# nebula-beta/MonocularSfM

Hardware: AMD Instinct MI355X
Metric: descriptor-pairs/sec (and image-pairs/sec); match-index bit-parity vs CPU (higher is better)
Workload: dtype f32

## Files before the change

monocularsfm_amd/csrc/msfm_job.hip.h:

```cpp
#pragma once

static int call_prologue(msfm_ctx* ctx) {
    HIPCHK(ctx, hipSetDevice(ctx->device));
    ctx->cur = &ctx->sc[0];
    for (Scratch& s : ctx->sc) forget_sweeps(ctx, s);
    if (!ctx->deferred.empty()) {
        HIPCHK(ctx, hipDeviceSynchronize());
        ctx->deferred.flush();
    }
    return settle_store(ctx);
}

template <class Attempt>
static int rerun_alone(msfm_ctx* ctx, Attempt attempt) {
    for (int k = 1;; ++k) {
        bool retry = false;
        const int rc = attempt(&retry);
        if (rc != MSFM_OK || !retry) return rc;
        if (k >= 6) return fail(ctx, MSFM_E_DEVICE, "batch kept overflowing its queues");
    }
}

struct MatchJob {
    msfm_ctx* ctx = nullptr;
    std::vector<int32_t> pairs_own;
    const int32_t* pairs = nullptr;
    int n_pairs = 0;
    msfm_match_params prm = {0.8f, 1, 0.7};
    PruneParams prune = {1, 0.8f, 0.7f};
    msfm_verify_params verify_store = {};
    const msfm_verify_params* verify = nullptr;
    bool streaming = false;
    bool select = false;
    bool pose = false;
    bool refine = false;
    hipEvent_t ev_begin = nullptr, ev_end = nullptr;
    int kSets = kInFlight;
    long long kScratchBytes = 1;
    MsfmRouteKnobs knobs = {};
    int kMaxPairsPerBatch = kDefaultMaxPairsPerBatch;
    std::vector<long long> marks;
    long long cost_done = 0;
    bool need_fix = false;
    SubBatch sb[kInFlight];
    int next_begin = 0;
    long long issued = 0, completed = 0;
    bool memory_wait = false;
    int memory_shrinks = 0;

    int start(msfm_ctx* c, const int32_t* pairs_in, int n, const msfm_match_params* params, const msfm_verify_params* vp, bool stream_mode) {
        ctx = c;
        pairs = pairs_in;
        n_pairs = n;
        streaming = stream_mode;
        verify = nullptr;
        c->have_results = c->sel_valid = c->tv_valid = false;
        select = vp && c->model_select && c->verify_model != MSFM_VERIFY_HOMOGRAPHY;
        c->sel_records.assign(select && !stream_mode ? 3 * (size_t)n : 0, 0);
        pose = vp && c->two_view && c->verify_model == MSFM_VERIFY_ESSENTIAL;
        c->tv_records.assign(pose && !stream_mode ? (size_t)n : 0, msfm_two_view_record{});
        c->tvr_valid = false;
        refine = pose && c->tv_refine;
        c->tvr_records.assign(refine && !stream_mode ? (size_t)n : 0, msfm_two_view_refinement{});
        if (vp) {
            verify_store = *vp;
            verify = &verify_store;
            c->staged_solved = 0;
            c->staged_rounds = 0;
        }
        for (SubBatch& w : sb) w = SubBatch{};
        next_begin = 0;
        issued = completed = 0;
        memory_wait = false;
        memory_shrinks = 0;
        ctx->last_hip_error = 0;
        prm = msfm_match_params{0.8f, 1, 0.7};
        if (params) prm = *params;
        prune = PruneParams{1, prm.ratio, (float)prm.max_distance};
        if ((double)prune.max_distance < prm.max_distance) prune.max_distance = nextafterf(prune.max_distance, __builtin_huge_valf());
        if (!(prm.ratio > 0.f) || !(prm.ratio <= 1.f)) prune.ratio = 0.f;
        if (!(prm.max_distance >= 0.0)) prune.max_distance = __builtin_huge_valf();
        int rc = call_prologue(ctx);
        if (rc != MSFM_OK) return rc;
        rc = rebuild_stale_twins(ctx, pairs, 2 * n_pairs);
        if (rc != MSFM_OK) return rc;
        ctx->res_offsets.assign((size_t)n_pairs + 1, 0);
        ctx->res_sens.assign((size_t)n_pairs, 0);
        ctx->res_count = 0;
        ctx->prof = msfm_profile{};
        ctx->out_used = 0;
        for (OutSeg& s : ctx->out_segs) s.count = 0;
        if (!streaming) {
            long long bound = 1;
            for (int k = 0; k < n_pairs; ++k) {
                const int i = pairs[2 * k], j = pairs[2 * k + 1];
                if (i < 0 || i >= kSlots || j < 0 || j >= kSlots) return fail(ctx, MSFM_E_INVALID, "image id out of range");
                const long long n1 = ctx->images[(size_t)i].n, n2 = ctx->images[(size_t)j].n;
                if (n1 > 0 && n2 > 0) bound += prm.cross_check ? std::min(n1, n2) : n1;
            }
            if (ctx->res_qt.reserve((size_t)bound * 8) != hipSuccess || ctx->res_dist.reserve((size_t)bound * 4) != hipSuccess)
                return fail(ctx, MSFM_E_DEVICE, "cannot reserve address space for the result lists");
        }

        ev_begin = get_event(ctx, 0), ev_end = get_event(ctx, 1);
        if (!ev_begin || !ev_end) return fail(ctx, MSFM_E_DEVICE, "hipEventCreate failed");
        HIPCHK(ctx, hipEventRecord(ev_begin, ctx->sc[0].stream));

        kSets = ctx->in_flight;
        long long budget = ctx->scratch_bytes > 0 ? ctx->scratch_bytes : kDefaultScratchBytes;
        if (ctx->budget_cached > 0 && ctx->budget_for_store == ctx->store.bytes() && ctx->budget_for_limit == ctx->scratch_bytes) {
            budget = ctx->budget_cached;
        } else {
            size_t free_b = 0, total_b = 0;
            if (hipMemGetInfo(&free_b, &total_b) == hipSuccess) {
                long long held = 0;
                for (Scratch& sc : ctx->sc) held += sc.device_bytes();
                const long long avail = (long long)free_b + held;
                budget = std::min(budget, ctx->scratch_bytes > 0 ? avail / 2 : avail / 4);
            }
            ctx->budget_cached = budget;
            ctx->budget_for_store = ctx->store.bytes();
            ctx->budget_for_limit = ctx->scratch_bytes;
        }
        kScratchBytes = std::max<long long>(1, budget / kSets);
        knobs = ctx->route_knobs();
        kMaxPairsPerBatch = ctx->max_pairs_per_batch;
        marks.clear();
        if (ctx->pipeline > 1 && n_pairs > 1) {
            long long total = 0;
            for (int k = 0; k < n_pairs; ++k) {
                const int i = pairs[2 * k], j = pairs[2 * k + 1];
                if (i < 0 || i >= kSlots || j < 0 || j >= kSlots) return fail(ctx, MSFM_E_INVALID, "image id out of range");
                const long long n1 = ctx->images[i].n, n2 = ctx->images[j].n;
                if (n1 > 0 && n2 > 0) total += n1 * n2;
            }
            marks = msfm_pipeline_marks(total, std::min<long long>(ctx->pipeline, total / kMinPipelineCost), ctx->pipeline_taper);
        }
        cost_done = 0;
        need_fix = !(prm.ratio <= 1.f);
        if (streaming) ctx->series_open = true;
        return MSFM_OK;
    }

    int build(SubBatch& w, int begin, const std::vector<char>& force_exact) {
        w.b = Batch{};
        w.begin = begin;
        if (begin == 0) cost_done = 0;
        const long long cost_begin = (begin == w.begin_of_cost) ? w.cost_begin : cost_done;
        w.begin_of_cost = begin;
        w.cost_begin = cost_begin;
        long long mark = 0;
        if (!marks.empty()) {
            size_t i = 0;
            while (i + 2 < marks.size() && cost_begin >= (marks[i] + marks[i + 1]) / 2) ++i;
            mark = marks[i + 1];
        }
        long long est = 0, cost = 0;
        int end = begin;
        while (end < n_pairs && (end - begin) < kMaxPairsPerBatch) {
            PairDesc pd;
            PfPair pp;
            int rc = fill_pair(ctx, pairs[2 * end], pairs[2 * end + 1], pd, pp);
            if (rc != MSFM_OK) return rc;
            const Image &ia = ctx->images[pairs[2 * end]], &ib = ctx->images[pairs[2 * end + 1]];
            if (verify && (ia.nk < ia.n || ib.nk < ib.n))
                return fail(ctx, MSFM_E_STATE, "geometric verification needs msfm_upload_keypoints for image " +
                                                   std::to_string(ia.nk < ia.n ? pairs[2 * end] : pairs[2 * end + 1]));
            const int route = msfm_scratch_route(knobs, prune.prune, prune.ratio, pp.use != 0, ia.is_u8, ib.is_u8);
            const long long need = pd.valid ? msfm_pair_scratch_bytes(pd.n1, pd.n2, pd.n1pad, pd.n2pad, pd.a_blocks, pd.a_blocks256, route, pose, refine) : 0;
            const long long c = pd.valid ? (long long)pd.n1 * pd.n2 : 0;
            if (end > begin && est + need > kScratchBytes) break;
            if (end > begin && !marks.empty() && cost_begin + cost + c / 2 > mark) break;
            est += need;
            cost += c;
            const size_t k = w.b.pairs.size();
            if (k < force_exact.size() && force_exact[k]) {
                pp.use = 0;
                pd.path = 0;
            }
            w.b.pairs.push_back(pd);
            w.b.pf.push_back(pp);
            w.b.id1.push_back(pairs[2 * end]);
            w.b.id2.push_back(pairs[2 * end + 1]);
            ++end;
        }
        w.end = end;
        cost_done = cost_begin + cost;
        return prepare_batch_images(ctx, w.b, prune);
    }

    int issue(SubBatch& w, size_t ev_base) {
        Batch& b = w.b;
        const size_t P = b.pairs.size();
        const int begin = w.begin;
        w.ev_base = ev_base;
        w.exact_launched = false;
        SC.prof = msfm_profile{};
        SC.seq = ctx->issue_seq++;
        SC.sweep2_recorded = false;
        int rc = run_knn(ctx, b, ev_base, &w.exact_launched, prune, need_fix, true);
        if (rc != MSFM_OK) return rc;
        const long long oe = std::max<long long>(1, b.out_elems);
        HIPCHK(ctx, SC.d_st_qt.ensure(oe * sizeof(int2)));
        HIPCHK(ctx, SC.d_st_d.ensure(oe * 4));
        HIPCHK(ctx, SC.d_sub_qt.ensure(oe * sizeof(int2)));
        HIPCHK(ctx, SC.d_sub_d.ensure(oe * 4));
        HIPCHK(ctx, SC.d_counts.ensure(P * 4));
        HIPCHK(ctx, SC.d_sens.ensure(P * 4));
        HIPCHK(ctx, SC.d_offsets.ensure((P + 1) * 8));
        EpiParams ep = {prm.ratio, prm.cross_check, prm.max_distance};
        if (SC.keys_epilogue)
            hipLaunchKernelGGL(epilogue_kernel<KnnFromKeys>, dim3((unsigned)P), dim3(256), 0, SC.stream, SC.d_pairs.as<PairDesc>(), ep,
                               KnnFromKeys{SC.d_tu.as<float>(), SC.d_best.as<unsigned long long>(), SC.d_second.as<unsigned long long>(),
                                           msfm_ratio_cap_on(prune.prune, prune.ratio) ? 1 : 0},
                               SC.d_st_qt.as<int2>(), SC.d_st_d.as<float>(), SC.d_counts.as<int>(), SC.d_sens.as<int>());
        else
            hipLaunchKernelGGL(epilogue_kernel<KnnFromArrays>, dim3((unsigned)P), dim3(256), 0, SC.stream, SC.d_pairs.as<PairDesc>(), ep,
                               KnnFromArrays{SC.d_k_i0.as<int>(), SC.d_k_d0.as<float>(), SC.d_k_d1.as<float>()},
                               SC.d_st_qt.as<int2>(), SC.d_st_d.as<float>(), SC.d_counts.as<int>(), SC.d_sens.as<int>());
        HIPCHK(ctx, hipGetLastError());
        const int* d_counts = SC.d_counts.as<int>();
        const int2* d_st_qt = SC.d_st_qt.as<int2>();
        const float* d_st_d = SC.d_st_d.as<float>();
        if (verify) {
            rc = issue_verify(b, begin, oe, ev_base);
            if (rc != MSFM_OK) return rc;
            d_counts = SC.d_counts2.as<int>();
            d_st_qt = SC.d_st2_qt.as<int2>();
            d_st_d = SC.d_st2_d.as<float>();
        }
        hipLaunchKernelGGL(scan_counts_kernel, dim3(1), dim3(256), 0, SC.stream, d_counts,
                           SC.d_offsets.as<long long>(), (int)P);
        HIPCHK(ctx, hipGetLastError());
        hipLaunchKernelGGL(gather_kernel, dim3((unsigned)P), dim3(256), 0, SC.stream, SC.d_pairs.as<PairDesc>(),
                           d_counts, SC.d_offsets.as<long long>(), d_st_qt,
                           d_st_d, SC.d_sub_qt.as<int2>(), SC.d_sub_d.as<float>());
        HIPCHK(ctx, hipGetLastError());
        rc = queue_tail_copies(ctx, P, select ? &SC.d_vs_records : nullptr);
        if (rc != MSFM_OK) return rc;
        if (pose) {
            const size_t rec_bytes = P * sizeof(msfm_two_view_record);
            HIPCHK(ctx, SC.h_tv.ensure(rec_bytes + (refine ? P * sizeof(msfm_two_view_refinement) : 0) + 64, 0));
            char* h = nullptr;
            HIPCHK(ctx, hipHostGetDevicePointer((void**)&h, SC.h_tv.p, 0));
            ExportSegs segs = {};
            segs.s[0] = ExportSeg{SC.d_tv_records.as<char>(), h, (unsigned)rec_bytes};
            if (refine)
                segs.s[1] = ExportSeg{SC.d_tvr_records.as<char>(), h + rec_bytes, (unsigned)(P * sizeof(msfm_two_view_refinement))};
            hipLaunchKernelGGL(export_tail_kernel, dim3(32), dim3(256), 0, SC.stream, segs);
            HIPCHK(ctx, hipGetLastError());
        }
        return MSFM_OK;
    }

    bool staged() const { return ctx->verify_model == MSFM_VERIFY_ESSENTIAL || ctx->verify_model == MSFM_VERIFY_HOMOGRAPHY; }

    int issue_verify(Batch& b, int begin, long long oe, size_t ev_base) {
        const size_t P = b.pairs.size();
        const int model = ctx->verify_model;
        std::vector<VerifyPair>& vpairs = b.verify_pairs;
        vpairs.resize(P);
        for (size_t p = 0; p < P; ++p)
            vpairs[p] = VerifyPair{ctx->images[pairs[2 * (begin + (int)p)]].kxy, ctx->images[pairs[2 * (begin + (int)p) + 1]].kxy};
        HIPCHK(ctx, SC.d_vf_pairs.ensure(P * sizeof(VerifyPair)));
        const bool e = model == MSFM_VERIFY_ESSENTIAL;
        for (DevBuf* xy : {e ? &SC.d_ve_x1 : &SC.d_vf_x1, e ? &SC.d_ve_y1 : &SC.d_vf_y1, e ? &SC.d_ve_x2 : &SC.d_vf_x2, e ? &SC.d_ve_y2 : &SC.d_vf_y2})
            HIPCHK(ctx, xy->ensure(oe * (e ? 8 : 4)));
        if (select && e)
            for (DevBuf* xy : {&SC.d_vf_x1, &SC.d_vf_y1, &SC.d_vf_x2, &SC.d_vf_y2}) HIPCHK(ctx, xy->ensure(oe * 4));
        if (!staged()) HIPCHK(ctx, SC.d_vf_flags.ensure(oe));
        HIPCHK(ctx, SC.d_vf_hyp.ensure(P * (size_t)verify->max_iters * 4));
        HIPCHK(ctx, SC.d_vf_best_it.ensure(P * 4));
        HIPCHK(ctx, SC.d_vf_best_count.ensure(P * 4));
        if (staged() || select) {
            HIPCHK(ctx, SC.d_staged_state.ensure((3 * P + 2) * 4));
            HIPCHK(ctx, SC.d_staged_stats.ensure(sizeof(StagedStats)));
        }
        if (select) HIPCHK(ctx, SC.d_vs_records.ensure(P * sizeof(SelectRecord)));
        HIPCHK(ctx, SC.d_st2_qt.ensure(oe * sizeof(int2)));
        HIPCHK(ctx, SC.d_st2_d.ensure(oe * 4));
        HIPCHK(ctx, SC.d_counts2.ensure(P * 4));
        HIPCHK(ctx, hipMemcpyAsync(SC.d_vf_pairs.p, vpairs.data(), P * sizeof(VerifyPair), hipMemcpyHostToDevice, SC.stream));
        if (staged() || select) {
            HIPCHK(ctx, hipMemsetAsync(SC.d_staged_state.p, 0, (3 * P + 2) * 4, SC.stream));
            HIPCHK(ctx, hipMemsetAsync(SC.d_staged_stats.p, 0, sizeof(StagedStats), SC.stream));
        }
        hipEvent_t v0 = get_event(ctx, ev_base + 6), v1 = get_event(ctx, ev_base + 7);
        if (!v0 || !v1) return fail(ctx, MSFM_E_DEVICE, "hipEventCreate failed");
        HIPCHK(ctx, hipEventRecord(v0, SC.stream));
        const PairDesc* dp = SC.d_pairs.as<PairDesc>();
        const VerifyPair* vp = SC.d_vf_pairs.as<VerifyPair>();
        const int* d_counts = SC.d_counts.as<int>();
        const int2* d_st_qt = SC.d_st_qt.as<int2>();
        const float* d_st_d = SC.d_st_d.as<float>();
        int* hyp = SC.d_vf_hyp.as<int>();
        const int* best_it = SC.d_vf_best_it.as<int>();
        if (model == MSFM_VERIFY_FUNDAMENTAL) {
            VerifyParams vprm = {verify->threshold * verify->threshold, verify->confidence, verify->max_iters, 0, verify->seed};
            float *x1 = SC.d_vf_x1.as<float>(), *y1 = SC.d_vf_y1.as<float>(), *x2 = SC.d_vf_x2.as<float>(), *y2 = SC.d_vf_y2.as<float>();
            hipLaunchKernelGGL(vf_points_kernel, dim3((unsigned)P), dim3(256), 0, SC.stream, dp, vp, d_counts, d_st_qt, x1, y1, x2, y2);
            HIPCHK(ctx, hipGetLastError());
            hipLaunchKernelGGL(vf_hypotheses_kernel, dim3((unsigned)((vprm.max_iters + 255) / 256), (unsigned)P), dim3(256), 0, SC.stream,
                               dp, d_counts, (const float*)x1, (const float*)y1, (const float*)x2, (const float*)y2, hyp, vprm);
            HIPCHK(ctx, hipGetLastError());
            hipLaunchKernelGGL(vf_select_kernel, dim3((unsigned)((P + 63) / 64)), dim3(64), 0, SC.stream, d_counts, (const int*)hyp, (int)P,
                               vprm, SC.d_vf_best_it.as<int>(), SC.d_vf_best_count.as<int>());
            HIPCHK(ctx, hipGetLastError());
            hipLaunchKernelGGL(vf_mask_compact_kernel, dim3((unsigned)P), dim3(256), 0, SC.stream, dp, d_counts, d_st_qt, d_st_d,
                               (const float*)x1, (const float*)y1, (const float*)x2, (const float*)y2, best_it,
                               (const int*)SC.d_vf_best_count.as<int>(), SC.d_vf_flags.as<unsigned char>(), vprm, SC.d_st2_qt.as<int2>(),
                               SC.d_st2_d.as<float>(), SC.d_counts2.as<int>());
        } else if (model == MSFM_VERIFY_ESSENTIAL) {
            const double f = (ctx->camera.fx + ctx->camera.fy) * 0.5, tn = verify->threshold / f;
            StagedParams prm = {tn * tn, verify->confidence, verify->max_iters, 0, verify->seed};
            double *x1 = SC.d_ve_x1.as<double>(), *y1 = SC.d_ve_y1.as<double>(), *x2 = SC.d_ve_x2.as<double>(), *y2 = SC.d_ve_y2.as<double>();
            hipLaunchKernelGGL(ve_points_kernel, dim3((unsigned)P), dim3(256), 0, SC.stream, dp, vp, d_counts, d_st_qt, ctx->camera, x1, y1, x2, y2);
            HIPCHK(ctx, hipGetLastError());
            int rc = issue_rounds<5, kVeRound>(P, kVeGroupsPerCU, prm, [&](unsigned grid, int* list, StagedStats* stats) {
                hipLaunchKernelGGL(ve_round_kernel, dim3(grid), dim3(kVeRound), 0, SC.stream, dp, d_counts, (const double*)x1, (const double*)y1,
                                   (const double*)x2, (const double*)y2, list, (int)P, hyp, prm, stats);
            });
            if (rc != MSFM_OK) return rc;
            hipLaunchKernelGGL(ve_mask_compact_kernel, dim3((unsigned)P), dim3(64), 0, SC.stream, dp, d_counts, d_st_qt, d_st_d, (const double*)x1,
                               (const double*)y1, (const double*)x2, (const double*)y2, best_it, prm, SC.d_st2_qt.as<int2>(),
                               SC.d_st2_d.as<float>(), SC.d_counts2.as<int>());
        } else {
            StagedParams prm = {verify->threshold * verify->threshold, verify->confidence, verify->max_iters, 0, verify->seed};
            float *x1 = SC.d_vf_x1.as<float>(), *y1 = SC.d_vf_y1.as<float>(), *x2 = SC.d_vf_x2.as<float>(), *y2 = SC.d_vf_y2.as<float>();
            hipLaunchKernelGGL(vf_points_kernel, dim3((unsigned)P), dim3(256), 0, SC.stream, dp, vp, d_counts, d_st_qt, x1, y1, x2, y2);
            HIPCHK(ctx, hipGetLastError());
            int rc = issue_rounds<4, kVhRound>(P, kVhGroupsPerCU, prm, [&](unsigned grid, int* list, StagedStats* stats) {
                hipLaunchKernelGGL(vh_round_kernel, dim3(grid), dim3(kVhRound), 0, SC.stream, dp, d_counts, (const float*)x1, (const float*)y1,
                                   (const float*)x2, (const float*)y2, list, (int)P, hyp, prm, stats);
            });
            if (rc != MSFM_OK) return rc;
            hipLaunchKernelGGL(vh_mask_compact_kernel, dim3((unsigned)P), dim3(64), 0, SC.stream, dp, d_counts, d_st_qt, d_st_d, (const float*)x1,
                               (const float*)y1, (const float*)x2, (const float*)y2, best_it, prm, SC.d_st2_qt.as<int2>(),
                               SC.d_st2_d.as<float>(), SC.d_counts2.as<int>());
        }
        HIPCHK(ctx, hipGetLastError());
        if (pose) {
            HIPCHK(ctx, SC.d_tv_records.ensure(P * sizeof(msfm_two_view_record)));
            HIPCHK(ctx, SC.d_tv_idx.ensure(oe * 4));
            HIPCHK(ctx, SC.d_tv_angles.ensure(oe * 8));
            if (select) {
                HIPCHK(ctx, SC.d_tv_best_it.ensure(P * 4));
                ExportSegs segs = {};
                segs.s[0] = ExportSeg{SC.d_vf_best_it.as<char>(), SC.d_tv_best_it.as<char>(), (unsigned)(P * 4)};
                hipLaunchKernelGGL(export_tail_kernel, dim3(32), dim3(256), 0, SC.stream, segs);
                HIPCHK(ctx, hipGetLastError());
            }
        }
        if (select) {
            const int rc = issue_select(P, dp, vp);
            if (rc != MSFM_OK) return rc;
        }
        if (pose) {
            const double f = (ctx->camera.fx + ctx->camera.fy) * 0.5, tn = verify->threshold / f;
            const StagedParams prm = {tn * tn, verify->confidence, verify->max_iters, 0, verify->seed};
            const unsigned grid = (unsigned)std::min<size_t>(P, (size_t)kTvGroupsPerCU * (size_t)std::max(1, ctx->cu_count));
            hipLaunchKernelGGL(tv_pose_kernel, dim3(grid), dim3(kTvThreads), 0, SC.stream, dp, d_counts, (const double*)SC.d_ve_x1.as<double>(),
                               (const double*)SC.d_ve_y1.as<double>(), (const double*)SC.d_ve_x2.as<double>(),
                               (const double*)SC.d_ve_y2.as<double>(), (const int*)(select ? SC.d_tv_best_it.as<int>() : SC.d_vf_best_it.as<int>()),
                               (const SelectRecord*)(select ? SC.d_vs_records.as<SelectRecord>() : nullptr), prm, f, ctx->tv_params, (int)P,
                               SC.d_tv_idx.as<int>(), SC.d_tv_angles.as<double>(), SC.d_tv_records.as<msfm_two_view_record>());
            HIPCHK(ctx, hipGetLastError());
            if (refine) {
                HIPCHK(ctx, SC.d_tvr_records.ensure(P * sizeof(msfm_two_view_refinement)));
                const unsigned rgrid = (unsigned)std::min<size_t>(P, (size_t)kTvrGroupsPerCU * (size_t)std::max(1, ctx->cu_count));
                hipLaunchKernelGGL(tv_refine_kernel, dim3(rgrid), dim3(kTvrThreads), 0, SC.stream, dp, (const double*)SC.d_ve_x1.as<double>(),
                                   (const double*)SC.d_ve_y1.as<double>(), (const double*)SC.d_ve_x2.as<double>(),
                                   (const double*)SC.d_ve_y2.as<double>(), (const int*)SC.d_tv_idx.as<int>(), f, ctx->tv_params,
                                   ctx->tvr_params, (int)P, SC.d_tv_angles.as<double>(), SC.d_tv_records.as<msfm_two_view_record>(),
                                   SC.d_tvr_records.as<msfm_two_view_refinement>());
                HIPCHK(ctx, hipGetLastError());
            }
        }
        HIPCHK(ctx, hipEventRecord(v1, SC.stream));
        return MSFM_OK;
    }

    int issue_select(size_t P, const PairDesc* dp, const VerifyPair* vp) {
        StagedParams prm = {verify->threshold * verify->threshold, verify->confidence, verify->max_iters, 0, verify->seed};
        const int* d_counts = SC.d_counts.as<int>();
        const int2* d_st_qt = SC.d_st_qt.as<int2>();
        const float* d_st_d = SC.d_st_d.as<float>();
        int* hyp = SC.d_vf_hyp.as<int>();
        float *x1 = SC.d_vf_x1.as<float>(), *y1 = SC.d_vf_y1.as<float>(), *x2 = SC.d_vf_x2.as<float>(), *y2 = SC.d_vf_y2.as<float>();
        if (ctx->verify_model == MSFM_VERIFY_ESSENTIAL) {
            hipLaunchKernelGGL(vf_points_kernel, dim3((unsigned)P), dim3(256), 0, SC.stream, dp, vp, d_counts, d_st_qt, x1, y1, x2, y2);
            HIPCHK(ctx, hipGetLastError());
        }
        HIPCHK(ctx, hipMemsetAsync(SC.d_staged_state.p, 0, (3 * P + 2) * 4, SC.stream));
        int rc = issue_rounds<4, kVhRound>(P, kVhGroupsPerCU, prm, [&](unsigned grid, int* list, StagedStats* stats) {
            hipLaunchKernelGGL(vh_round_kernel, dim3(grid), dim3(kVhRound), 0, SC.stream, dp, d_counts, (const float*)x1, (const float*)y1,
                               (const float*)x2, (const float*)y2, list, (int)P, hyp, prm, stats);
        });
        if (rc != MSFM_OK) return rc;
        hipLaunchKernelGGL(two_view_select_kernel, dim3((unsigned)P), dim3(64), 0, SC.stream, dp, d_counts, d_st_qt, d_st_d, (const float*)x1,
                           (const float*)y1, (const float*)x2, (const float*)y2, (const int*)SC.d_vf_best_it.as<int>(), prm, ctx->verify_model,
                           ctx->h_ratio, SC.d_st2_qt.as<int2>(), SC.d_st2_d.as<float>(), SC.d_counts2.as<int>(),
                           SC.d_vs_records.as<SelectRecord>());
        HIPCHK(ctx, hipGetLastError());
        return MSFM_OK;
    }

    template <int kSample, int kRound, class LaunchRound>
    int issue_rounds(size_t P, int groups_per_cu, StagedParams& prm, LaunchRound launch_round) {
        StagedStats* stats = SC.d_staged_stats.as<StagedStats>();
        int* state = SC.d_staged_state.as<int>();
        int* list = state + P;
        const int rounds = (prm.max_iters + kRound - 1) / kRound;
        const unsigned grid = (unsigned)std::min<size_t>(P, (size_t)groups_per_cu * (size_t)std::max(1, ctx->cu_count));
        for (int r = -1; r < rounds; ++r) {
            prm.round = r;
            if (r >= 0) {
                launch_round(grid, list, stats);
                HIPCHK(ctx, hipGetLastError());
            }
            hipLaunchKernelGGL((staged_decide_kernel<kSample, kRound>), dim3((unsigned)((P + 63) / 64)), dim3(64), 0, SC.stream,
                               (const int*)SC.d_counts.as<int>(), (const int*)SC.d_vf_hyp.as<int>(), (int)P, prm, state, list,
                               SC.d_vf_best_it.as<int>(), SC.d_vf_best_count.as<int>(), stats);
            HIPCHK(ctx, hipGetLastError());
        }
        return MSFM_OK;
    }

    int complete(SubBatch& w, std::vector<char>& force_exact, bool* retry_out) {
        Batch& b = w.b;
        const size_t P = b.pairs.size();
        *retry_out = false;
        HIPCHK(ctx, hipStreamSynchronize(SC.stream));
        bool retry = false, retry_pf = false;
        force_exact.resize(P, 0);
        int rc = check_fix_overflow(ctx, &retry);
        if (rc != MSFM_OK) return rc;
        rc = finish_prefilter(ctx, b, force_exact, &retry_pf);
        if (rc != MSFM_OK) return rc;
        if (retry || retry_pf) {
            ctx->prof.tie_queue_regrows += SC.prof.tie_queue_regrows;
            ctx->prof.plan_regrows += SC.prof.plan_regrows;
            ctx->prof.fallback_pairs += SC.prof.fallback_pairs;
            *retry_out = true;
            return MSFM_OK;
        }
        SC.prof.fallback_pairs = 0;
        const char* h = SC.h_tail.as<char>();
        const long long* offs = reinterpret_cast<const long long*>(h + 8);
        const int32_t* sens = reinterpret_cast<const int32_t*>(h + 8 + (P + 1) * 8);
        const long long total = offs[P];
        const size_t base = streaming ? 0 : ctx->res_count;
        if (ctx->tracks.open && !ctx->tracks.closed && !ctx->tracks.suppress && !ctx->tracks.add_only) {
            rc = tk_fold_sub_batch(ctx, SC, b.id1.data(), b.id2.data(), P, offs);
            if (rc != MSFM_OK) return rc;
        }
        if (streaming) {
            HIPCHK(ctx, SC.h_sub_qt.ensure(((size_t)total + 1) * 8, 0));
            HIPCHK(ctx, SC.h_sub_d.ensure(((size_t)total + 1) * 4, 0));
            if (total > 0) {
                HIPCHK(ctx, hipMemcpyAsync(SC.h_sub_qt.p, SC.d_sub_qt.p, (size_t)total * 8, hipMemcpyDeviceToHost, SC.stream));
                HIPCHK(ctx, hipMemcpyAsync(SC.h_sub_d.p, SC.d_sub_d.p, (size_t)total * 4, hipMemcpyDeviceToHost, SC.stream));
                HIPCHK(ctx, hipStreamSynchronize(SC.stream));
            }
            w.offsets.assign(offs, offs + P + 1);
            w.sens.assign(sens, sens + P);
            if (select) w.sel.assign(sens + P, sens + 4 * P);
            else w.sel.clear();
            if (pose) w.tv.assign(SC.h_tv.as<msfm_two_view_record>(), SC.h_tv.as<msfm_two_view_record>() + P);
            else w.tv.clear();
            w.tvr.clear();
            if (refine) {
                const msfm_two_view_refinement* h_tvr = reinterpret_cast<const msfm_two_view_refinement*>(SC.h_tv.as<msfm_two_view_record>() + P);
                w.tvr.assign(h_tvr, h_tvr + P);
            }
            for (size_t p = 0; p < P; ++p) SC.prof.order_sensitive_rows += sens[p];
            ctx->res_count += (size_t)total;
        } else {
            const size_t need = base + (size_t)total + 1;
            if (ctx->res_qt.ensure_pinned(need * 8) != hipSuccess || ctx->res_dist.ensure_pinned(need * 4) != hipSuccess)
                return fail(ctx, MSFM_E_DEVICE, "cannot page-lock the result lists (beyond the reserved range or the host's memory): use msfm_match_pairs_begin / _next");
            if (total > 0) {
                OutSeg* seg = ctx->out_used ? &ctx->out_segs[ctx->out_used - 1] : nullptr;
                if (!seg || seg->cap - seg->count < (size_t)total) {
                    while (true) {
                        if (ctx->out_used == ctx->out_segs.size()) {
                            ctx->out_segs.push_back(OutSeg{});
                            OutSeg& s = ctx->out_segs.back();
                            const size_t cap = std::max<size_t>((size_t)total * 8, (size_t)4 << 20);
                            HIPCHK(ctx, s.qt.ensure(cap * 8));
                            HIPCHK(ctx, s.d.ensure(cap * 4));
                            s.cap = cap;
                        }
                        seg = &ctx->out_segs[ctx->out_used++];
                        seg->first = base;
                        seg->count = 0;
                        if (seg->cap >= (size_t)total) break;
                    }
                }
                HIPCHK(ctx, ctx->res_qt.copy_in(base * 8, SC.d_sub_qt.p, (size_t)total * 8, SC.stream));
                HIPCHK(ctx, ctx->res_dist.copy_in(base * 4, SC.d_sub_d.p, (size_t)total * 4, SC.stream));
                HIPCHK(ctx, hipMemcpyAsync(seg->qt.as<int2>() + seg->count, SC.d_sub_qt.p, (size_t)total * 8, hipMemcpyDeviceToDevice, SC.stream));
                HIPCHK(ctx, hipMemcpyAsync(seg->d.as<float>() + seg->count, SC.d_sub_d.p, (size_t)total * 4, hipMemcpyDeviceToDevice, SC.stream));
                seg->count += (size_t)total;
            }
            ctx->res_count = base + (size_t)total;
            for (size_t p = 0; p < P; ++p) {
                ctx->res_offsets[(size_t)w.begin + p + 1] = (int64_t)base + offs[p + 1];
                ctx->res_sens[(size_t)w.begin + p] = sens[p];
                SC.prof.order_sensitive_rows += sens[p];
            }
            if (select) std::memcpy(ctx->sel_records.data() + 3 * (size_t)w.begin, sens + P, P * 12);
            if (pose) std::memcpy(ctx->tv_records.data() + (size_t)w.begin, SC.h_tv.p, P * sizeof(msfm_two_view_record));
            if (refine)
                std::memcpy(ctx->tvr_records.data() + (size_t)w.begin, SC.h_tv.as<msfm_two_view_record>() + P, P * sizeof(msfm_two_view_refinement));
        }
        SC.prof.descriptor_pairs += b.desc_pairs;
        SC.prof.dist_algo_bytes += b.algo_bytes;
        rc = accumulate_kernel_time(ctx, w.ev_base, w.exact_launched);
        if (rc != MSFM_OK) return rc;
        if (verify) {
            float vms = 0.f;
            HIPCHK(ctx, hipEventElapsedTime(&vms, ctx->ev_pool[w.ev_base + 6], ctx->ev_pool[w.ev_base + 7]));
            SC.prof.verify_ms += vms;
            if (staged() || select) {
                StagedStats st = {};
                HIPCHK(ctx, hipMemcpyAsync(&st, SC.d_staged_stats.p, sizeof(st), hipMemcpyDeviceToHost, SC.stream));
                HIPCHK(ctx, hipStreamSynchronize(SC.stream));
                ctx->staged_solved += (long long)st.solved;
                ctx->staged_rounds = std::max(ctx->staged_rounds, st.rounds);
            }
        }
        SC.prof.sub_batches += 1;
        add_profile(ctx->prof, SC.prof);
        return MSFM_OK;
    }

// ... 103 lines not shown
```

monocularsfm_amd/csrc/msfm_kernels.hip.h:

```cpp
#pragma once
#include <hip/hip_runtime.h>
#include <stdint.h>
#include "msfm_hostutil.h"

#pragma clang fp contract(off)

namespace msfm {

constexpr int kDim = 128;
constexpr int kBM = 128;
constexpr int kBN = 128;
constexpr int kTM = 8;
constexpr int kTN = 4;
constexpr int kThreads = 512;
constexpr int kChunkPos = 32;
constexpr int kChunks = kDim / kChunkPos;
constexpr int kPanelFloats = kBM * kDim;
constexpr int kSlotFloats = kChunkPos * kBN;
constexpr int kWaveCols = kBN / 8;
constexpr int kWaveSlotFloats = kChunkPos * kWaveCols;
constexpr int kLdsA = 0;
constexpr int kLdsB = kPanelFloats;
constexpr int kLdsFloats = kLdsB + 8 * 2 * kWaveSlotFloats;
constexpr int kLdsBytes = kLdsFloats * 4;
// ... 170 lines not shown
template <int ORDER>
__global__ __launch_bounds__(kThreads) void dist_top2_kernel(
    const PairDesc* __restrict__ pairs, const WorkItem* __restrict__ items,
    float* __restrict__ rp_s0, int* __restrict__ rp_i0, float* __restrict__ rp_s1,
    float* __restrict__ cp_s0, int* __restrict__ cp_i0, float* __restrict__ cp_s1) {
    using OT = OrderTraits<ORDER>;
    extern __shared__ __attribute__((aligned(16))) float smem[];
    float* sA = smem + kLdsA;

    const WorkItem item = items[blockIdx.x];
    if (item.pair < 0) return;
    const PairDesc pd = pairs[item.pair];

    const int tid = threadIdx.x;
    const int lane = tid & 63;
    const int wave = __builtin_amdgcn_readfirstlane(tid >> 6);
    const int ty = lane & 15;
    const int tx = lane >> 4;
    float* sBw = smem + kLdsB + wave * (2 * kWaveSlotFloats);

    const int n_steps = (item.bt_end - item.bt_begin) * kChunks;
    const float* gB = pd.b_panel + (size_t)item.bt_begin * kPanelFloats + wave * kWaveCols + (lane >> 2) * kBN + (lane & 3) * 4;
    auto dma_chunk = [&](int st) {
        const float* g = gB + (size_t)st * kSlotFloats;
        float* l = sBw + (st & 1) * kWaveSlotFloats;
        __builtin_amdgcn_global_load_lds((const __attribute__((address_space(1))) void*)g,
                                         (__attribute__((address_space(3))) void*)l, 16, 0, 0);
        __builtin_amdgcn_global_load_lds((const __attribute__((address_space(1))) void*)(g + 16 * kBN),
                                         (__attribute__((address_space(3))) void*)(l + 256), 16, 0, 0);
    };

    glds_copy(pd.a_panel + (size_t)item.a_blk * kPanelFloats, sA, kPanelFloats, tid);
    dma_chunk(0);
    __syncthreads();

    const int arow0 = item.a_blk * kBM + 4 * ty;
    float r_s0[kTM], r_s1[kTM];
    int r_i0[kTM];
#pragma unroll
    for (int i = 0; i < kTM; ++i) { r_s0[i] = f_inf(); r_s1[i] = f_inf(); r_i0[i] = -1; }
    constexpr bool kStashIdx = OT::kGroups == 16;
    int* sIdx = reinterpret_cast<int*>(smem + kLdsFloats);
    if (kStashIdx) {
#pragma unroll
        for (int i = 0; i < kTM; ++i) sIdx[i * kThreads + tid] = -1;
    }

    v2f lvl0[4][kTN], lvl1[4][kTN], lvl2[4][kTN];
    (void)lvl2;

    int step = 0;
    auto begin_chunk = [&](int c, const float*& sa, const float*& sb) {
        asm volatile("s_waitcnt vmcnt(0)" ::: "memory");
        if (step + 1 < n_steps) dma_chunk(step + 1);
        sa = sA + c * kChunkPos * kBM + 4 * ty;
        sb = sBw + (step & 1) * kWaveSlotFloats + 4 * tx;
        ++step;
    };
#define MSFM_FOREACH(expr)                       \
    _Pragma("unroll") for (int i = 0; i < 4; ++i) \
        _Pragma("unroll") for (int j = 0; j < kTN; ++j) { expr; }

#pragma unroll 1
    for (int bt = item.bt_begin; bt < item.bt_end; ++bt) {
        const float *sa, *sb;
        if (OT::kGroups == 4) {
#pragma unroll 1
            for (int c = 0; c < kChunks; ++c) {
                begin_chunk(c, sa, sb);
                v2f s[4][kTN];
                group_chains<ORDER>(sa, sb, s);
                if ((c & 1) == 0) { MSFM_FOREACH(lvl0[i][j] = s[i][j]) }
                else if (c == 1) { MSFM_FOREACH(lvl1[i][j] = lvl0[i][j] + s[i][j]) }
                else { MSFM_FOREACH(lvl1[i][j] = lvl1[i][j] + (lvl0[i][j] + s[i][j])) }
            }
        } else if (OT::kGroups == 16) {
#pragma unroll 1
            for (int c = 0; c < kChunks; ++c) {
                begin_chunk(c, sa, sb);
                v2f s[4][kTN], q[4][kTN];
                group_chains<ORDER>(sa, sb, lvl0);
                group_chains<ORDER>(sa + OT::kGroupPos * kBM, sb + OT::kGroupPos * kWaveCols, s);
                MSFM_FOREACH(q[i][j] = lvl0[i][j] + s[i][j])
                group_chains<ORDER>(sa + 2 * OT::kGroupPos * kBM, sb + 2 * OT::kGroupPos * kWaveCols, lvl0);
                group_chains<ORDER>(sa + 3 * OT::kGroupPos * kBM, sb + 3 * OT::kGroupPos * kWaveCols, s);
                MSFM_FOREACH(q[i][j] = q[i][j] + (lvl0[i][j] + s[i][j]))
                if (c == 0 || c == 2) { MSFM_FOREACH(lvl1[i][j] = q[i][j]) }
                else if (c == 1) { MSFM_FOREACH(lvl2[i][j] = lvl1[i][j] + q[i][j]) }
                else { MSFM_FOREACH(lvl2[i][j] = lvl2[i][j] + (lvl1[i][j] + q[i][j])) }
            }
        } else {
#pragma unroll 1
            for (int c = 0; c < kChunks; ++c) {
                begin_chunk(c, sa, sb);
                group_chains<ORDER>(sa, sb, lvl0);
                v2f s[4][kTN];
                group_chains<ORDER>(sa + OT::kGroupPos * kBM, sb + OT::kGroupPos * kWaveCols, s);
                if (c == 0 || c == 2) { MSFM_FOREACH(lvl1[i][j] = lvl0[i][j] + s[i][j]) }
                else if (c == 1) { MSFM_FOREACH(lvl2[i][j] = lvl1[i][j] + (lvl0[i][j] + s[i][j])) }
                else { MSFM_FOREACH(lvl2[i][j] = lvl2[i][j] + (lvl1[i][j] + (lvl0[i][j] + s[i][j]))) }
            }
        }
        float fin[kTM][kTN];
#pragma unroll
        for (int i = 0; i < kTM; ++i)
#pragma unroll
            for (int j = 0; j < kTN; ++j)
                fin[i][j] = fminf((OT::kGroups == 4) ? lvl1[i >> 1][j][i & 1] : lvl2[i >> 1][j][i & 1], f_inf());

        const int col0 = bt * kBN + wave * kWaveCols + tx * kTN;
        if ((bt + 1) * kBN > pd.n2 || (item.a_blk + 1) * kBM > pd.n1) {
#pragma unroll
            for (int i = 0; i < kTM; ++i)
#pragma unroll
                for (int j = 0; j < kTN; ++j)
                    if (arow0 + (i & 3) + (i >> 2) * 64 >= pd.n1 || col0 + j >= pd.n2) fin[i][j] = f_inf();
        }
        if (kStashIdx) {
#pragma unroll
            for (int i = 0; i < kTM; ++i) r_i0[i] = sIdx[i * kThreads + tid];
        }
#pragma unroll
        for (int i = 0; i < kTM; ++i)
#pragma unroll
            for (int j = 0; j < kTN; ++j) top2_push(r_s0[i], r_i0[i], r_s1[i], fin[i][j], col0 + j);
        if (kStashIdx) {
#pragma unroll
            for (int i = 0; i < kTM; ++i) sIdx[i * kThreads + tid] = r_i0[i];
        }
#pragma unroll
        for (int j = 0; j < kTN; ++j) {
            float c_s0 = f_inf(), c_s1 = f_inf();
            int c_i0 = -1;
#pragma unroll
            for (int i = 0; i < kTM; ++i)
                top2_push(c_s0, c_i0, c_s1, fin[i][j], arow0 + (i & 3) + (i >> 2) * 64);
#pragma unroll
            for (int m = 1; m < 16; m <<= 1) {
                const float o_s0 = __shfl_xor(c_s0, m);
                const int o_i0 = __shfl_xor(c_i0, m);
                const float o_s1 = __shfl_xor(c_s1, m);
                top2_merge(c_s0, c_i0, c_s1, o_s0, o_i0, o_s1);
            }
            if (ty == 0) {
                const long long o = pd.cp_off + (long long)item.a_blk * pd.n2pad + col0 + j;
                cp_s0[o] = c_s0;
                cp_i0[o] = c_i0;
                cp_s1[o] = c_s1;
            }
        }
    }

    if (kStashIdx) {
#pragma unroll
        for (int i = 0; i < kTM; ++i) r_i0[i] = sIdx[i * kThreads + tid];
    }
#pragma unroll
    for (int i = 0; i < kTM; ++i) {
#pragma unroll
        for (int m = 16; m < 64; m <<= 1) {
            const float o_s0 = __shfl_xor(r_s0[i], m);
            const int o_i0 = __shfl_xor(r_i0[i], m);
            const float o_s1 = __shfl_xor(r_s1[i], m);
            top2_merge(r_s0[i], r_i0[i], r_s1[i], o_s0, o_i0, o_s1);
        }
    }
    __syncthreads();
    float* sR = smem + kLdsB;
    if (tx == 0) {
#pragma unroll
        for (int i = 0; i < kTM; ++i) {
            const int r = 4 * ty + (i & 3) + (i >> 2) * 64;
            sR[(wave * 3 + 0) * kBM + r] = r_s0[i];
            sR[(wave * 3 + 1) * kBM + r] = __int_as_float(r_i0[i]);
            sR[(wave * 3 + 2) * kBM + r] = r_s1[i];
        }
    }
    __syncthreads();
    if (tid < kBM) {
        float s0 = sR[0 * kBM + tid];
        int i0 = __float_as_int(sR[1 * kBM + tid]);
        float s1 = sR[2 * kBM + tid];
#pragma unroll
        for (int w = 1; w < 8; ++w)
            top2_merge(s0, i0, s1, sR[(w * 3 + 0) * kBM + tid], __float_as_int(sR[(w * 3 + 1) * kBM + tid]),
                       sR[(w * 3 + 2) * kBM + tid]);
        const long long o = pd.rp_off + (long long)item.range * pd.n1pad + item.a_blk * kBM + tid;
        rp_s0[o] = s0;
        rp_i0[o] = i0;
        rp_s1[o] = s1;
    }
#undef MSFM_FOREACH
}

__global__ void merge_knn_kernel(const PairDesc* __restrict__ pairs,
                                 const float* __restrict__ rp_s0, const int* __restrict__ rp_i0,
                                 const float* __restrict__ rp_s1, const float* __restrict__ cp_s0,
                                 const int* __restrict__ cp_i0, const float* __restrict__ cp_s1,
                                 int* __restrict__ k_i0, float* __restrict__ k_d0, float* __restrict__ k_d1,
                                 int* __restrict__ fix_count, int4* __restrict__ fix_list, int fix_cap) {
    MSFM_TAIL_PRIO();
    const PairDesc pd = pairs[blockIdx.y];
    if (!pd.valid || pd.path != 0) return;
    const int e = blockIdx.x * blockDim.x + threadIdx.x;
    for (int dir = 0; dir < 2; ++dir) {
        const int n = dir == 0 ? pd.n1 : pd.n2;
        if (e >= n) continue;
        const int npad = dir == 0 ? pd.n1pad : pd.n2pad;
        const int parts = dir == 0 ? pd.ranges : pd.a_blocks;
        const long long base = (dir == 0 ? pd.rp_off : pd.cp_off) + e;
        const float* ps0 = dir == 0 ? rp_s0 : cp_s0;
        const int* pi0 = dir == 0 ? rp_i0 : cp_i0;
        const float* ps1 = dir == 0 ? rp_s1 : cp_s1;
        float s0 = ps0[base], s1 = ps1[base];
        int i0 = pi0[base];
        for (int p = 1; p < parts; ++p) {
            const long long o = base + (long long)p * npad;
            top2_merge(s0, i0, s1, ps0[o], pi0[o], ps1[o]);
        }
        const float d0 = (s0 < f_inf()) ? sqrtf(s0) : 3.402823466e+38f;
        const float d1 = (s1 < f_inf()) ? sqrtf(s1) : 3.402823466e+38f;
        if (!(s0 < f_inf())) i0 = -1;
        const long long ko = (dir == 0 ? pd.kf_off : pd.kr_off) + e;
        k_i0[ko] = i0;
        k_d0[ko] = d0;
        k_d1[ko] = d1;
        if (i0 >= 0 && d0 == d1) {
            const int slot = atomicAdd(fix_count, 1);
            if (slot < fix_cap) fix_list[slot] = make_int4((int)blockIdx.y, dir, e, 0);
        }
    }
}

__device__ __forceinline__ int tie_rawp_pos(int k) { return 64 * (k >> 6) + 4 * (k & 15) + ((k >> 4) & 3); }

template <int ORDER>
__device__ float l2sqr_rowmajor(const float* __restrict__ a, const float* __restrict__ b) {
    using OT = OrderTraits<ORDER>;
    float lvl[5] = {0.f, 0.f, 0.f, 0.f, 0.f};
    for (int g = 0; g < OT::kGroups; ++g) {
        float s = 0.f;
        for (int v = 0; v < 4; ++v) {
            float p = 0.f;
            for (int it = 0; it < OT::kIters; ++it) {
                const int k = tie_rawp_pos(OT::pos_to_k(g * OT::kGroupPos + v * OT::kIters + it));
                const float t = a[k] - b[k];
                if (it == 0) p = t * t;
                else if (OT::kFused) p = __builtin_fmaf(t, t, p);
                else p = p + t * t;
            }
            s = (v == 0) ? p : s + p;
        }
        int j = 0;
        for (int gg = g; gg & 1; gg >>= 1, ++j) s = lvl[j] + s;
        lvl[j] = s;
    }
    return lvl[OT::kGroups == 4 ? 2 : (OT::kGroups == 8 ? 3 : 4)];
}

template <int ORDER>
__global__ void tie_fixup_kernel(const PairDesc* __restrict__ pairs, const int* __restrict__ fix_count,
                                 const int4* __restrict__ fix_list, int fix_cap,
                                 int* __restrict__ k_i0, const float* __restrict__ k_d0) {
    MSFM_TAIL_PRIO();
    const int nfix = min(*fix_count, fix_cap);
    for (int f = blockIdx.x; f < nfix; f += gridDim.x) {
        const int4 w = fix_list[f];
        const PairDesc pd = pairs[w.x];
        const bool fwd = (w.y == 0);
        const float* me = (fwd ? pd.a_rawp : pd.b_rawp) + (size_t)w.z * kDim;
        const float* other = fwd ? pd.b_rawp : pd.a_rawp;
        const int n_other = fwd ? pd.n2 : pd.n1;
        const long long ko = (fwd ? pd.kf_off : pd.kr_off) + w.z;
        const float d0 = k_d0[ko];
        int best = 0x7fffffff;
        for (int t = threadIdx.x; t < n_other; t += 64) {
            const float s = fwd ? l2sqr_rowmajor<ORDER>(me, other + (size_t)t * kDim)
                                : l2sqr_rowmajor<ORDER>(other + (size_t)t * kDim, me);
            if (sqrtf(s) == d0) { best = t; break; }
        }
#pragma unroll
        for (int m = 32; m >= 1; m >>= 1) best = min(best, __shfl_xor(best, m));
        if (threadIdx.x == 0 && best != 0x7fffffff) k_i0[ko] = best;
    }
}

struct EpiParams {
    float ratio;
    int cross_check;
    double max_distance;
};

__device__ __forceinline__ bool order_sensitive(int i0, float d0, float d1, float ratio, double max_distance, bool forward) {
    return msfm_order_sensitive(i0, d0, d1, ratio, max_distance, forward);
}
__device__ __forceinline__ bool lowe_keep(int i0, float d0, float d1, float ratio) {
    return (i0 >= 0) && (d1 < kNoNeighbour || d1 == f_inf()) && (d0 < ratio * d1);
}

struct KnnFromArrays {
    const int* i0;
    const float* d0;
    const float* d1;
    __device__ __forceinline__ void get(long long slot, bool , int& i, float& a, float& b) const {
        i = i0[slot];
        a = d0[slot];
        b = d1[slot];
    }
};
struct KnnFromKeys {
    const float* tuv;
    const unsigned long long* best;
    const unsigned long long* second;
    int cap;
    __device__ __forceinline__ void get(long long slot, bool reverse, int& i, float& a, float& b) const {
        i = -1;
        a = b = kNoNeighbour;
        if (tuv[slot] == -f_inf()) return;
        const unsigned long long kb = best[slot], ks = second[slot];
        if (kb != ~0ull) { i = (int)(unsigned)(kb & 0xffffffffu); a = sqrtf(__uint_as_float((unsigned)(kb >> 32))); }
        if (ks != ~0ull) b = sqrtf(__uint_as_float((unsigned)(ks >> 32)));
        else if (cap && reverse && kb != ~0ull) b = f_inf();
    }
};

template <class KNN>
__global__ __launch_bounds__(256) void epilogue_kernel(const PairDesc* __restrict__ pairs, EpiParams prm, KNN knn,
                                                       int2* __restrict__ st_qt, float* __restrict__ st_d,
                                                       int* __restrict__ counts, int* __restrict__ sens_counts) {
    MSFM_TAIL_PRIO();
    const PairDesc pd = pairs[blockIdx.x];
    __shared__ int wsum[4];
    __shared__ int running, n_sens;
    if (threadIdx.x == 0) { running = 0; n_sens = 0; }
    __syncthreads();
    if (!pd.valid || pd.n2 < 2 || (prm.cross_check && pd.n1 < 2)) {
        if (threadIdx.x == 0) { counts[blockIdx.x] = 0; sens_counts[blockIdx.x] = 0; }
        return;
    }
    const bool certify = !pd.exact_int;
    const int lane = threadIdx.x & 63, wave = threadIdx.x >> 6;
    for (int q0 = 0; q0 < pd.n1; q0 += 256) {
        const int q = q0 + threadIdx.x;
        bool keep = false, sens = false;
        int t = -1;
        float d0 = 0.f;
        if (q < pd.n1) {
            float d1;
            knn.get(pd.kf_off + q, false, t, d0, d1);
            keep = lowe_keep(t, d0, d1, prm.ratio);
            sens = certify && order_sensitive(t, d0, d1, prm.ratio, prm.max_distance, true);
            if (keep && prm.cross_check) {
                int rq;
                float rd0, rd1;
                knn.get(pd.kr_off + t, true, rq, rd0, rd1);
                const bool rkeep = lowe_keep(rq, rd0, rd1, prm.ratio);
                const int vis = rkeep ? rq : 0;
                keep = (vis == q);
            }
            if (keep && ((double)d0 > prm.max_distance)) keep = false;
        }
        const unsigned long long sb = __ballot(sens);
        if (lane == 0 && sb) atomicAdd(&n_sens, __popcll(sb));
        const unsigned long long bal = __ballot(keep);
        const int before = __popcll(bal & ((1ull << lane) - 1ull));
        if (lane == 0) wsum[wave] = __popcll(bal);
        __syncthreads();
        int off = running;
        for (int w = 0; w < wave; ++w) off += wsum[w];
        if (keep) {
            st_qt[pd.out_off + off + before] = make_int2(q, t);
            st_d[pd.out_off + off + before] = d0;
        }
        __syncthreads();
        if (threadIdx.x == 0) running += wsum[0] + wsum[1] + wsum[2] + wsum[3];
        __syncthreads();
    }
    if (certify && prm.cross_check)
        for (int t0 = 0; t0 < pd.n2; t0 += 256) {
            const int t = t0 + threadIdx.x;
            int ri = -1;
            float rd0 = 0.f, rd1 = 0.f;
            if (t < pd.n2) knn.get(pd.kr_off + t, true, ri, rd0, rd1);
            const bool s = t < pd.n2 && order_sensitive(ri, rd0, rd1, prm.ratio, prm.max_distance, false);
            const unsigned long long sb = __ballot(s);
            if (lane == 0 && sb) atomicAdd(&n_sens, __popcll(sb));
        }
    __syncthreads();
    if (threadIdx.x == 0) { counts[blockIdx.x] = running; sens_counts[blockIdx.x] = n_sens; }
}

__global__ void scan_counts_kernel(const int* __restrict__ counts, long long* __restrict__ offsets, int n) {
    MSFM_TAIL_PRIO();
    __shared__ long long carry;
    __shared__ long long wtot[4];
    if (threadIdx.x == 0) carry = 0;
    __syncthreads();
    const int lane = threadIdx.x & 63, wave = threadIdx.x >> 6;
    for (int base = 0; base < n; base += 256) {
        const int i = base + threadIdx.x;
        long long v = (i < n) ? counts[i] : 0;
        long long incl = v;
#pragma unroll
        for (int m = 1; m < 64; m <<= 1) {
            const long long o = __shfl_up(incl, m);
            if (lane >= m) incl += o;
        }
        if (lane == 63) wtot[wave] = incl;
        __syncthreads();
        long long woff = carry;
        for (int w = 0; w < wave; ++w) woff += wtot[w];
        if (i < n) offsets[i] = woff + incl - v;
        __syncthreads();
        if (threadIdx.x == 0) carry += wtot[0] + wtot[1] + wtot[2] + wtot[3];
        __syncthreads();
    }
    if (threadIdx.x == 0) offsets[n] = carry;
}

__global__ void gather_kernel(const PairDesc* __restrict__ pairs, const int* __restrict__ counts,
                              const long long* __restrict__ offsets, const int2* __restrict__ st_qt,
                              const float* __restrict__ st_d, int2* __restrict__ out_qt,
                              float* __restrict__ out_d) {
    MSFM_TAIL_PRIO();
    const PairDesc pd = pairs[blockIdx.x];
    const int c = counts[blockIdx.x];
    const long long o = offsets[blockIdx.x];
    for (int i = threadIdx.x; i < c; i += blockDim.x) {
        out_qt[o + i] = st_qt[pd.out_off + i];
        out_d[o + i] = st_d[pd.out_off + i];
    }
}

}
```

Measured before the change: 6231 billion.

## Batch epilogue loads across passes and fold count scan into gather

The epilogue kernel now handles four 256-element passes per iteration. It issues all forward, reverse-certify and cross-check KNN loads up front, pinned in registers, so their memory latency overlaps. It also merges the separate reverse order-sensitivity loop into the same pass and replaces per-wave shared atomics with a per-thread count reduced at the end. The single-block scan kernel is removed: each gather block now computes its own prefix offset by summing the counts of all earlier pairs. That saves a launch and a serial scan but costs O(P^2) total reads of the counts array when P is large.

Result: no change. 6227 billion, median of 3 (-0.1%).

```diff
diff --git a/monocularsfm_amd/csrc/msfm_job.hip.h b/monocularsfm_amd/csrc/msfm_job.hip.h
--- a/monocularsfm_amd/csrc/msfm_job.hip.h
+++ b/monocularsfm_amd/csrc/msfm_job.hip.h
@@ -229,9 +229,6 @@
             d_st_qt = SC.d_st2_qt.as<int2>();
             d_st_d = SC.d_st2_d.as<float>();
         }
-        hipLaunchKernelGGL(scan_counts_kernel, dim3(1), dim3(256), 0, SC.stream, d_counts,
-                           SC.d_offsets.as<long long>(), (int)P);
-        HIPCHK(ctx, hipGetLastError());
         hipLaunchKernelGGL(gather_kernel, dim3((unsigned)P), dim3(256), 0, SC.stream, SC.d_pairs.as<PairDesc>(),
                            d_counts, SC.d_offsets.as<long long>(), d_st_qt,
                            d_st_d, SC.d_sub_qt.as<int2>(), SC.d_sub_d.as<float>());
diff --git a/monocularsfm_amd/csrc/msfm_kernels.hip.h b/monocularsfm_amd/csrc/msfm_kernels.hip.h
--- a/monocularsfm_amd/csrc/msfm_kernels.hip.h
+++ b/monocularsfm_amd/csrc/msfm_kernels.hip.h
@@ -496,10 +496,18 @@
     const int* i0;
     const float* d0;
     const float* d1;
-    __device__ __forceinline__ void get(long long slot, bool , int& i, float& a, float& b) const {
-        i = i0[slot];
-        a = d0[slot];
-        b = d1[slot];
+    struct Raw {
+        int i;
+        float a, b;
+    };
+    __device__ __forceinline__ Raw head(long long slot) const { return Raw{i0[slot], d0[slot], d1[slot]}; }
+    __device__ __forceinline__ bool more(const Raw& ) const { return false; }
+    __device__ __forceinline__ void rest(long long , Raw& ) const {}
+    __device__ __forceinline__ void pin(Raw& r) const { asm volatile("" : "+v"(r.i), "+v"(r.a), "+v"(r.b)); }
+    __device__ __forceinline__ void value(const Raw& r, bool , int& i, float& a, float& b) const {
+        i = r.i;
+        a = r.a;
+        b = r.b;
     }
 };
 struct KnnFromKeys {
@@ -507,16 +515,29 @@
     const unsigned long long* best;
     const unsigned long long* second;
     int cap;
-    __device__ __forceinline__ void get(long long slot, bool reverse, int& i, float& a, float& b) const {
+    struct Raw {
+        float tu;
+        unsigned long long kb, ks;
+    };
+    __device__ __forceinline__ Raw head(long long slot) const { return Raw{tuv[slot], ~0ull, ~0ull}; }
+    __device__ __forceinline__ bool more(const Raw& r) const { return r.tu != -f_inf(); }
+    __device__ __forceinline__ void rest(long long slot, Raw& r) const {
+        r.kb = best[slot];
+        r.ks = second[slot];
+    }
+    __device__ __forceinline__ void pin(Raw& r) const { asm volatile("" : "+v"(r.tu), "+v"(r.kb), "+v"(r.ks)); }
+    __device__ __forceinline__ void value(const Raw& r, bool reverse, int& i, float& a, float& b) const {
         i = -1;
         a = b = kNoNeighbour;
-        if (tuv[slot] == -f_inf()) return;
-        const unsigned long long kb = best[slot], ks = second[slot];
+        if (r.tu == -f_inf()) return;
+        const unsigned long long kb = r.kb, ks = r.ks;
         if (kb != ~0ull) { i = (int)(unsigned)(kb & 0xffffffffu); a = sqrtf(__uint_as_float((unsigned)(kb >> 32))); }
         if (ks != ~0ull) b = sqrtf(__uint_as_float((unsigned)(ks >> 32)));
         else if (cap && reverse && kb != ~0ull) b = f_inf();
     }
 };
+
+constexpr int kEpiPasses = 4;
 
 template <class KNN>
 __global__ __launch_bounds__(256) void epilogue_kernel(const PairDesc* __restrict__ pairs, EpiParams prm, KNN knn,
@@ -524,103 +545,136 @@
                                                        int* __restrict__ counts, int* __restrict__ sens_counts) {
     MSFM_TAIL_PRIO();
     const PairDesc pd = pairs[blockIdx.x];
-    __shared__ int wsum[4];
-    __shared__ int running, n_sens;
-    if (threadIdx.x == 0) { running = 0; n_sens = 0; }
-    __syncthreads();
+    __shared__ int wsum[kEpiPasses][4];
+    __shared__ int n_sens;
     if (!pd.valid || pd.n2 < 2 || (prm.cross_check && pd.n1 < 2)) {
         if (threadIdx.x == 0) { counts[blockIdx.x] = 0; sens_counts[blockIdx.x] = 0; }
         return;
     }
+    if (threadIdx.x == 0) n_sens = 0;
+    __syncthreads();
     const bool certify = !pd.exact_int;
+    const bool rev_certify = certify && prm.cross_check;
     const int lane = threadIdx.x & 63, wave = threadIdx.x >> 6;
-    for (int q0 = 0; q0 < pd.n1; q0 += 256) {
-        const int q = q0 + threadIdx.x;
-        bool keep = false, sens = false;
-        int t = -1;
-        float d0 = 0.f;
-        if (q < pd.n1) {
-            float d1;
-            knn.get(pd.kf_off + q, false, t, d0, d1);
-            keep = lowe_keep(t, d0, d1, prm.ratio);
-            sens = certify && order_sensitive(t, d0, d1, prm.ratio, prm.max_distance, true);
-            if (keep && prm.cross_check) {
+    const int span = max(pd.n1, rev_certify ? pd.n2 : 0);
+    int running = 0;
+    int my_sens = 0;
+    for (int r0 = 0; r0 < span; r0 += kEpiPasses * 256) {
+        typename KNN::Raw fr[kEpiPasses], cr[kEpiPasses], rr[kEpiPasses];
+#pragma unroll
+        for (int k = 0; k < kEpiPasses; ++k) {
+            const int e = r0 + (int)threadIdx.x + 256 * k;
+            fr[k] = knn.head(pd.kf_off + min(e, pd.n1 - 1));
+            cr[k] = knn.head(pd.kr_off + (rev_certify ? min(e, pd.n2 - 1) : 0));
+        }
+#pragma unroll
+        for (int k = 0; k < kEpiPasses; ++k) {
+            const int e = r0 + (int)threadIdx.x + 256 * k;
+            knn.rest(pd.kf_off + ((e < pd.n1 && knn.more(fr[k])) ? e : 0), fr[k]);
+            knn.rest(pd.kr_off + ((rev_certify && e < pd.n2 && knn.more(cr[k])) ? e : 0), cr[k]);
+        }
+#pragma unroll
+        for (int k = 0; k < kEpiPasses; ++k) {
+            knn.pin(fr[k]);
+            knn.pin(cr[k]);
+        }
+        bool keep[kEpiPasses];
+        int t[kEpiPasses];
+        float d0[kEpiPasses];
+#pragma unroll
+        for (int k = 0; k < kEpiPasses; ++k) {
+            const int q = r0 + (int)threadIdx.x + 256 * k;
+            keep[k] = false;
+            t[k] = -1;
+            d0[k] = 0.f;
+            if (q < pd.n1) {
+                float d1;
+                knn.value(fr[k], false, t[k], d0[k], d1);
+                keep[k] = lowe_keep(t[k], d0[k], d1, prm.ratio);
+                if (certify && order_sensitive(t[k], d0[k], d1, prm.ratio, prm.max_distance, true)) ++my_sens;
+            }
+        }
+        if (prm.cross_check) {
+#pragma unroll
+            for (int k = 0; k < kEpiPasses; ++k) {
+                const long long slot = pd.kr_off + (keep[k] ? t[k] : 0);
+                rr[k] = knn.head(slot);
+                knn.rest(slot, rr[k]);
+            }
+#pragma unroll
+            for (int k = 0; k < kEpiPasses; ++k) knn.pin(rr[k]);
+        }
+#pragma unroll
+        for (int k = 0; k < kEpiPasses; ++k) {
+            const int q = r0 + (int)threadIdx.x + 256 * k;
+            if (keep[k] && prm.cross_check) {
                 int rq;
                 float rd0, rd1;
-                knn.get(pd.kr_off + t, true, rq, rd0, rd1);
+                knn.value(rr[k], true, rq, rd0, rd1);
                 const bool rkeep = lowe_keep(rq, rd0, rd1, prm.ratio);
                 const int vis = rkeep ? rq : 0;
-                keep = (vis == q);
-            }
-            if (keep && ((double)d0 > prm.max_distance)) keep = false;
-        }
-        const unsigned long long sb = __ballot(sens);
-        if (lane == 0 && sb) atomicAdd(&n_sens, __popcll(sb));
-        const unsigned long long bal = __ballot(keep);
-        const int before = __popcll(bal & ((1ull << lane) - 1ull));
-        if (lane == 0) wsum[wave] = __popcll(bal);
+                keep[k] = (vis == q);
+            }
+            if (keep[k] && ((double)d0[k] > prm.max_distance)) keep[k] = false;
+            if (rev_certify && q < pd.n2) {
+                int ri;
+                float rd0, rd1;
+                knn.value(cr[k], true, ri, rd0, rd1);
+                if (order_sensitive(ri, rd0, rd1, prm.ratio, prm.max_distance, false)) ++my_sens;
+            }
+        }
+        int before[kEpiPasses];
+#pragma unroll
+        for (int k = 0; k < kEpiPasses; ++k) {
+            const unsigned long long bal = __ballot(keep[k]);
+            before[k] = __popcll(bal & ((1ull << lane) - 1ull));
+            if (lane == 0) wsum[k][wave] = __popcll(bal);
+        }
         __syncthreads();
-        int off = running;
-        for (int w = 0; w < wave; ++w) off += wsum[w];
-        if (keep) {
-            st_qt[pd.out_off + off + before] = make_int2(q, t);
-            st_d[pd.out_off + off + before] = d0;
+#pragma unroll
+        for (int k = 0; k < kEpiPasses; ++k) {
+            int off = running;
+#pragma unroll
+            for (int w = 0; w < 4; ++w) {
+                const int v = wsum[k][w];
+                if (w < wave) off += v;
+                running += v;
+            }
+            if (keep[k]) {
+                st_qt[pd.out_off + off + before[k]] = make_int2(r0 + (int)threadIdx.x + 256 * k, t[k]);
+                st_d[pd.out_off + off + before[k]] = d0[k];
+            }
         }
         __syncthreads();
-        if (threadIdx.x == 0) running += wsum[0] + wsum[1] + wsum[2] + wsum[3];
-        __syncthreads();
-    }
-    if (certify && prm.cross_check)
-        for (int t0 = 0; t0 < pd.n2; t0 += 256) {
-            const int t = t0 + threadIdx.x;
-            int ri = -1;
-            float rd0 = 0.f, rd1 = 0.f;
-            if (t < pd.n2) knn.get(pd.kr_off + t, true, ri, rd0, rd1);
-            const bool s = t < pd.n2 && order_sensitive(ri, rd0, rd1, prm.ratio, prm.max_distance, false);
-            const unsigned long long sb = __ballot(s);
-            if (lane == 0 && sb) atomicAdd(&n_sens, __popcll(sb));
-        }
+    }
+#pragma unroll
+    for (int m = 32; m >= 1; m >>= 1) my_sens += __shfl_xor(my_sens, m);
+    if (lane == 0 && my_sens) atomicAdd(&n_sens, my_sens);
     __syncthreads();
     if (threadIdx.x == 0) { counts[blockIdx.x] = running; sens_counts[blockIdx.x] = n_sens; }
 }
 
-__global__ void scan_counts_kernel(const int* __restrict__ counts, long long* __restrict__ offsets, int n) {
+__global__ __launch_bounds__(256) void gather_kernel(const PairDesc* __restrict__ pairs, const int* __restrict__ counts,
+                                                     long long* __restrict__ offsets, const int2* __restrict__ st_qt,
+                                                     const float* __restrict__ st_d, int2* __restrict__ out_qt,
+                                                     float* __restrict__ out_d) {
     MSFM_TAIL_PRIO();
-    __shared__ long long carry;
     __shared__ long long wtot[4];
-    if (threadIdx.x == 0) carry = 0;
+    const int p = blockIdx.x;
+    const PairDesc pd = pairs[p];
+    const int c = counts[p];
+    long long o = 0;
+    for (int i = threadIdx.x; i < p; i += 256) o += counts[i];
+#pragma unroll
+    for (int m = 32; m >= 1; m >>= 1) o += __shfl_xor(o, m);
+    if ((threadIdx.x & 63) == 0) wtot[threadIdx.x >> 6] = o;
     __syncthreads();
-    const int lane = threadIdx.x & 63, wave = threadIdx.x >> 6;
-    for (int base = 0; base < n; base += 256) {
-        const int i = base + threadIdx.x;
-        long long v = (i < n) ? counts[i] : 0;
-        long long incl = v;
-#pragma unroll
-        for (int m = 1; m < 64; m <<= 1) {
-            const long long o = __shfl_up(incl, m);
-            if (lane >= m) incl += o;
-        }
-        if (lane == 63) wtot[wave] = incl;
-        __syncthreads();
-        long long woff = carry;
-        for (int w = 0; w < wave; ++w) woff += wtot[w];
-        if (i < n) offsets[i] = woff + incl - v;
-        __syncthreads();
-        if (threadIdx.x == 0) carry += wtot[0] + wtot[1] + wtot[2] + wtot[3];
-        __syncthreads();
-    }
-    if (threadIdx.x == 0) offsets[n] = carry;
-}
-
-__global__ void gather_kernel(const PairDesc* __restrict__ pairs, const int* __restrict__ counts,
-                              const long long* __restrict__ offsets, const int2* __restrict__ st_qt,
-                              const float* __restrict__ st_d, int2* __restrict__ out_qt,
-                              float* __restrict__ out_d) {
-    MSFM_TAIL_PRIO();
-    const PairDesc pd = pairs[blockIdx.x];
-    const int c = counts[blockIdx.x];
-    const long long o = offsets[blockIdx.x];
-    for (int i = threadIdx.x; i < c; i += blockDim.x) {
+    o = wtot[0] + wtot[1] + wtot[2] + wtot[3];
+    if (threadIdx.x == 0) {
+        offsets[p] = o;
+        if (p == (int)gridDim.x - 1) offsets[p + 1] = o + c;
+    }
+    for (int i = threadIdx.x; i < c; i += 256) {
         out_qt[o + i] = st_qt[pd.out_off + i];
         out_d[o + i] = st_d[pd.out_off + i];
     }
```
